# Hydrology-IFH/roger

Measured on AMD Instinct MI355X. Metric: cell-timesteps/sec on SVAT_benchmark grid, higher is better.
Workload: dtype f64

## Files before the change

include/roger_hip.h:

```cpp
#ifndef ROGER_HIP_H
#define ROGER_HIP_H

#include <stddef.h>
#include <stdint.h>

#ifdef __cplusplus
extern "C" {
#endif

#define RH_ABI_VERSION 6
#define RH_SLOTS_PER_DAY 144

typedef enum rh_status {
    RH_OK = 0,
    RH_ERR_ARG = -1,
    RH_ERR_HIP = -2,
    RH_ERR_STATE = -3,
    RH_ERR_NODEVICE = -4
} rh_status;

typedef enum rh_plane {
#define RH_FIELD_1(name) RH_P_##name,
#define RH_FIELD_2(name) RH_P_##name, RH_P_##name##_m1,
#define RH_FIELD(name, type, levels) RH_FIELD_##levels(name)
// ... 81 lines not shown
int rh_snow(rh_ctx *ctx);
int rh_infiltration(rh_ctx *ctx);
int rh_subsurface_runoff(rh_ctx *ctx);
int rh_surface_routing(rh_ctx *ctx);
int rh_subsurface_routing(rh_ctx *ctx);
int rh_step_routed(rh_ctx *ctx, int monthly);
int rh_route_out(rh_ctx *ctx, int which);
int rh_route_in(rh_ctx *ctx, int which);
int rh_route_get_edges(rh_ctx *ctx, int which, double *q_lo, double *q_hi);
int rh_route_get_static_edges(rh_ctx *ctx, int32_t *flow_dir_lo, int32_t *flow_dir_hi, int32_t *mask_lo, int32_t *mask_hi);
int rh_route_set_halo(rh_ctx *ctx, int side, const double *q, const int32_t *flow_dir, const int32_t *mask);
int rh_capillary_rise(rh_ctx *ctx);
int rh_storage(rh_ctx *ctx);
int rh_num_error(rh_ctx *ctx);
int rh_after_timestep(rh_ctx *ctx);
int rh_step_core(rh_ctx *ctx);

int rh_step_phase1(rh_ctx *ctx);
int rh_step_phase2(rh_ctx *ctx);
int rh_step_phase3(rh_ctx *ctx, int monthly);
int rh_svat_step(rh_ctx *ctx, int monthly);
int rh_svat_step_scalars(rh_ctx *ctx, int monthly, rh_scalars *s);
int rh_param_stats(rh_ctx *ctx, double *derived_fraction, double *uniform_bytes_per_cell);
int rh_step_summary(rh_ctx *ctx);
int rh_step_finish(rh_ctx *ctx, int monthly);
int rh_step_summary_expand(rh_ctx *ctx, int32_t *dev_dst64);
int rh_step_finish_compress(rh_ctx *ctx, int monthly, const int32_t *dev_src64);
int rh_set_forcing_stations(rh_ctx *ctx, const double *prec, const double *ta, const double *pet, const int64_t *year, const int64_t *month,
                            const int64_t *doy, int64_t nitt_forc, int n_stations, const int32_t *station_index);
int rh_hooks_phase(rh_ctx *ctx);
int rh_run_steps(rh_ctx *ctx, int64_t nsteps);
int rh_plane_is_pure_output(int model, int plane);
int rh_set_time_limit(rh_ctx *ctx, int64_t t_end);
int64_t rh_sparse_steps(const rh_ctx *ctx);
void *rh_predicate_words(rh_ctx *ctx);
int rh_predicates_expand(rh_ctx *ctx, int word, int32_t *dev_dst64);
int rh_predicates_compress(rh_ctx *ctx, int word, const int32_t *dev_src64);

int rh_comm_unique_id(void *id128);
int rh_comm_init(rh_ctx *ctx, const void *id128, int nranks, int rank);
int rh_set_comm(rh_ctx *ctx, void *nccl_comm);
int rh_comm_set_grid(rh_ctx *ctx, int px, int py);
int rh_comm_info(rh_ctx *ctx, int *nranks, int *rank);
int rh_run_steps_dist(rh_ctx *ctx, int64_t nsteps);

int rh_diag_configure(rh_ctx *ctx, const int *rate_planes, int n_rate, const int *collect_planes, int n_collect, int n_slots);
// ... 26 lines not shown
```

roger_amd/_native.py:

```python
import ctypes as C
import os

import numpy as np

PKG = os.path.dirname(os.path.abspath(__file__))
LIB_PATH = os.environ.get("ROGER_HIP_LIB", os.path.join(PKG, "libroger_hip.so"))


ABI_VERSION = 6


class RhConfig(C.Structure):
    _fields_ = [("nx", C.c_int64), ("ny", C.c_int64), ("device", C.c_int32), ("enable_lateral_flow", C.c_int32)] + [
        (k, C.c_double) for k in (
            "pi", "r_mp", "l_sc", "sf", "ta_fm", "rmax", "transp_water_stress", "atol", "rtol", "clay_min",
            "clay_max", "theta_rew_min", "theta_rew_max", "rew_min", "rew_max", "z_evap_max", "zroot_to_zsoil_max",
            "a_bc", "b_bc")
    ] + [("end_event", C.c_int64), ("hpi", C.c_int64), ("dx", C.c_double), ("placement_probes", C.c_int32), ("enable_routing_1D", C.c_int32),
         ("dy", C.c_double)]


class RhScalars(C.Structure):
    _fields_ = [
        ("itt", C.c_int64), ("time", C.c_int64), ("dt_secs", C.c_int64), ("itt_day", C.c_int64),
# ... 103 lines not shown
    lib.rh_step_routed.argtypes = [vp, i32]
    lib.rh_planes_held.argtypes = [vp]
    lib.rh_route_out.argtypes = [vp, i32]
    lib.rh_route_in.argtypes = [vp, i32]
    lib.rh_route_get_edges.argtypes = [vp, i32, vp, vp]
    lib.rh_route_get_static_edges.argtypes = [vp, vp, vp, vp, vp]
    lib.rh_route_set_halo.argtypes = [vp, i32, vp, vp, vp]
    lib.rh_diag_set_interval.argtypes = [vp, i64]
    lib.rh_diag_slot_times.argtypes = [vp, i32, C.POINTER(C.c_int64), C.POINTER(C.c_int64)]
    lib.rh_step_summary_expand.argtypes = [vp, vp]
    lib.rh_step_finish_compress.argtypes = [vp, i32, vp]
    lib.rh_set_forcing_weights.argtypes = [vp, vp, vp, vp]
    lib.rh_diag_configure.argtypes = [vp, vp, i32, vp, i32, i32]
    lib.rh_diag_download.argtypes = [vp, i32, i32, vp, C.c_size_t]
    lib.rh_diag_steps.argtypes = [vp, i32, C.POINTER(C.c_int64)]
    lib.rh_diag_device_ptr.argtypes = [vp, i32, i32]
    lib.rh_diag_device_ptr.restype = vp
    lib.rh_points_configure.argtypes = [vp, vp, i32, vp, i32, i64]
    lib.rh_points_count.argtypes = [vp, C.POINTER(C.c_int64)]
    lib.rh_points_read.argtypes = [vp, i64, i64, vp, vp, C.c_size_t]
    lib.rh_svat_step.argtypes = [vp, i32]
    lib.rh_svat_step_scalars.argtypes = [vp, i32, C.POINTER(RhScalars)]
    lib.rh_param_stats.argtypes = [vp, C.POINTER(C.c_double), C.POINTER(C.c_double)]
    lib.rh_run_steps.argtypes = [vp, i64]
    lib.rh_set_forcing_series.argtypes = [vp, vp, vp, vp, vp, vp, vp, i64]
    lib.rh_predicates_expand.argtypes = [vp, i32, vp]
    lib.rh_predicates_compress.argtypes = [vp, i32, vp]
    lib.rh_calibrate_copy.argtypes = [vp, i32, i32, i32]
    lib.rh_selftest_pow.argtypes = [vp, vp, vp, i64]
    lib.rh_selftest_window_sum.argtypes = [vp, vp, i64, vp]
    lib.rh_debug_swap_arenas.argtypes = [vp, vp]
    lib.rh_predicate_words.argtypes = [vp]
    lib.rh_predicate_words.restype = vp
    lib.rh_timing_summary.argtypes = [vp, C.POINTER(C.c_double), C.POINTER(C.c_int64)]
    lib.rh_timing_detail.argtypes = [vp, C.POINTER(C.c_double), C.POINTER(C.c_int32), C.c_int64, C.POINTER(C.c_int64)]
    lib.rh_enable_timing.argtypes = [vp, i32]
    _declare_sas(lib)
    _lib = lib
    return lib


class RhSasConfig(C.Structure):
    _fields_ = [("n_cells", C.c_int64), ("ages", C.c_int32), ("substeps", C.c_int32), ("device", C.c_int32),
                ("forcing_days", C.c_int32), ("age_statistics", C.c_int32), ("keep_distributions", C.c_int32),
                ("vsmow", C.c_double), ("d18O_min", C.c_double), ("d18O_max", C.c_double),
                ("tracer", C.c_int32), ("solver", C.c_int32)]
# ... 184 lines not shown


def sas_selftest_pow(x, k):
    lib = load()
    x = np.ascontiguousarray(x, dtype=np.float64)
    k = np.ascontiguousarray(np.broadcast_to(k, x.shape), dtype=np.float64)
    out = np.empty_like(x)
    rc = lib.rh_sas_selftest_pow(x.ctypes.data_as(C.c_void_p), k.ctypes.data_as(C.c_void_p), out.ctypes.data_as(C.c_void_p), x.size)
    if rc != 0:
        raise NativeError(f"rh_sas_selftest_pow failed ({rc})")
    return out


DAILY_INPUTS = ("inf_mat_rz", "inf_pf_rz", "inf_pf_ss", "evap_soil", "transp", "q_rz", "q_ss", "cpr_rz", "C_in")


DECLARED_SYMBOLS = (
    "rh_default_config", "rh_create", "rh_destroy", "rh_last_error", "rh_abi_version", "rh_set_stream", "rh_sync",
    "rh_num_planes", "rh_plane_name", "rh_plane_is_int", "rh_plane_index", "rh_num_cells", "rh_upload",
    "rh_download", "rh_plane_device_ptr", "rh_set_scalars", "rh_get_scalars", "rh_set_luts", "rh_set_forcing_day",
    "rh_topo", "rh_params_surface", "rh_params_soil", "rh_initial_conditions", "rh_adaptive_dt", "rh_interception",
    "rh_evapotranspiration", "rh_snow", "rh_infiltration", "rh_subsurface_runoff", "rh_capillary_rise",
    "rh_storage", "rh_num_error", "rh_after_timestep", "rh_step_phase1", "rh_step_phase2", "rh_step_phase3",
    "rh_svat_step", "rh_svat_step_scalars", "rh_param_stats", "rh_predicate_words", "rh_timing_summary", "rh_timing_detail", "rh_enable_timing", "rh_set_forcing_series",
    "rh_hooks_phase", "rh_run_steps", "rh_predicates_expand", "rh_predicates_compress", "rh_step_core", "rh_calibrate_copy", "rh_debug_swap_arenas", "rh_selftest_pow", "rh_selftest_window_sum", "rh_set_lut_mlms", "rh_params_lateral",
    "rh_step_summary", "rh_step_finish", "rh_diag_set_interval", "rh_diag_slot_times", "rh_placement_report", "rh_step_summary_expand", "rh_step_finish_compress", "rh_diag_configure", "rh_diag_download", "rh_diag_device_ptr", "rh_diag_steps",
    "rh_set_forcing_weights", "rh_adaptive_dt_finish", "rh_diag_upload", "rh_diag_set_slot_state", "rh_set_forcing_stations", "rh_step_mode", "rh_comm_unique_id", "rh_comm_init", "rh_set_comm", "rh_comm_info", "rh_comm_set_grid", "rh_plane_is_pure_output", "rh_sparse_steps", "rh_set_time_limit", "rh_run_steps_dist",
    "rh_surface_routing", "rh_subsurface_routing", "rh_step_routed", "rh_planes_held", "rh_route_out", "rh_route_in", "rh_route_get_edges", "rh_route_get_static_edges", "rh_route_set_halo",
    "rh_points_configure", "rh_points_count", "rh_points_read",
)


def selftest_window_sum(v144, itd):
    lib = load()
    v = np.ascontiguousarray(v144, dtype=np.float64)
    t = np.ascontiguousarray(itd, dtype=np.int64)
    if v.size != 144:
        raise ValueError("selftest_window_sum: a series of 144 slots")
    out = np.empty(2 * t.size, dtype=np.float64)
    rc = lib.rh_selftest_window_sum(v.ctypes.data_as(C.c_void_p), t.ctypes.data_as(C.c_void_p), t.size, out.ctypes.data_as(C.c_void_p))
    if rc != 0:
        raise NativeError(f"rh_selftest_window_sum failed ({rc})")
    return out[0::2], out[1::2]


def selftest_pow(x, y):
    lib = load()
# ... 237 lines not shown
        return n.value

    def points_read(self, first, n):
        n = int(n)
        nv, nc = getattr(self, "_points_shape", (0, 0))
        hdr = np.empty((n, 3), dtype=np.int64)
        values = np.empty((n, nv, nc), dtype=np.float64)
        self._check(self._lib.rh_points_read(self._h, int(first), n, hdr.ctypes.data_as(C.c_void_p), values.ctypes.data_as(C.c_void_p),
                                             values.nbytes), "rh_points_read")
        return hdr, values

    def pure_output_planes(self):
        model = 2 if self.routing else int(self.lateral)
        return [nm for nm, p in self.index.items() if self._lib.rh_plane_is_pure_output(model, p) == 1]

    def set_time_limit(self, t_end):
        self._check(self._lib.rh_set_time_limit(self._h, -1 if t_end is None else int(t_end)), "rh_set_time_limit")

    def param_stats(self):
        d, u = C.c_double(), C.c_double()
        self._check(self._lib.rh_param_stats(self._h, C.byref(d), C.byref(u)), "rh_param_stats")
        return d.value, u.value

    def sparse_steps(self):
        return int(self._lib.rh_sparse_steps(self._h))

    def step_mode(self):
        m = self._lib.rh_step_mode(self._h)
        return bool(m & 1), bool(m & 2)

    def comm_init(self, unique_id, nranks, rank):
        buf = C.create_string_buffer(bytes(unique_id), 128)
        self._check(self._lib.rh_comm_init(self._h, buf, int(nranks), int(rank)), "rh_comm_init")

    def comm_init_torch(self, group=None):
        import torch.distributed as dist

        rank, world = (dist.get_rank(group), dist.get_world_size(group)) if dist.is_initialized() else (0, 1)
        box = [comm_unique_id() if rank == 0 else None]
        if world > 1:
            dist.broadcast_object_list(box, src=0, group=group)
        self.comm_init(box[0], world, rank)

    def comm_info(self):
        n, r = C.c_int(), C.c_int()
        self._check(self._lib.rh_comm_info(self._h, C.byref(n), C.byref(r)), "rh_comm_info")
# ... 58 lines not shown
```

roger_amd/csrc/rh_context.h:

```cpp
#pragma once
struct DeviceHolds {
    bool pmask_valid = false;
    bool rot_consistent = false, m1_stale = false;
    bool summary_valid = false;
    bool routed_summary = false;
    bool exch_valid = false;
    bool pending_valid = false;
    bool pre_valid = false;
    int pending_hooks = 0;
    bool sparse_next = false;
    bool outputs_stale = false;
    bool last_sparse = false;
    bool agg_daily_stale = true;
    bool pred_daily_stale = true;
    bool front_daily_stale = true;
    int last_front = 0;
};

struct Switches {
    bool lazy_ok, sparse_ok, tail_ok, routed_device_ok, defer_select_ok, cell_front_ok;
    int64_t cell_front_max, cell_agg_split_min;
    int pmask_flags, placement_probes;
};
static Switches read_switches(const rh_config &cfg) {
    auto unset = [](const char *name) { return std::getenv(name) == nullptr; };
    auto number = [](const char *name, long long dflt) { const char *v = std::getenv(name); return v ? std::atoll(v) : dflt; };
    Switches s;
    s.lazy_ok = unset("RH_NO_LAZY_ROTATION");
    s.sparse_ok = unset("RH_NO_SPARSE_STORES");
    s.tail_ok = unset("RH_NO_TAIL_CTRL");
    s.routed_device_ok = unset("RH_ROUTED_BY_ROUTINE");
    s.defer_select_ok = unset("RH_NO_DEFERRED_SELECT");
    s.cell_front_ok = unset("RH_PER_CELL_OLD_FRONT") && s.defer_select_ok;
    s.cell_front_max = number("RH_CELL_FRONT_MAX", 2097152);
    s.cell_agg_split_min = number("RH_CELL_AGG_SPLIT_MIN", 65536);
    s.pmask_flags = (unset("RH_NO_PARAM_UNIFORM") ? 1 : 0) | (unset("RH_NO_PARAM_DERIVE") ? 2 : 0) | (unset("RH_NO_MASK_CONSTANT") ? 4 : 0);
    s.placement_probes = (int)number("RH_PLACEMENT_PROBES", cfg.placement_probes);
    return s;
}

struct rh_ctx {
    Stream stream;
    rh_config cfg = {};
    int64_t n = 0;
    Arena arena = {};
    DevBuf<char> arena_mem;
    DevBuf<DevState> dev;
    PinnedBlock<HostExport> hexp;
    unsigned long long hexp_seq = 0;
    DevBuf<unsigned long long> pmask_buf;
    DevBuf<double> forc_cell_buf[3];
    DevBuf<double> weight_buf[3];
    DevBuf<int> station_buf;
    DevBuf<double> forc_multi_buf;
    DevBuf<double> transpose_buf;
    DevBuf<double> agg_cell_buf;
    DevBuf<char> series_buf;
    DevBuf<double> mlms_buf;
    DevBuf<void> stage_buf;
    bool per_cell = false;
    bool forcing_set = false;
    DeviceHolds held;
    Switches sw;
    int n_groups = 1;
    bool obs_reads_m1 = false;
    bool obs_reads_sparse = false;
    int64_t t_end = -1;
    int64_t call_sparse_steps = 0;
    DevBuf<double> diag_buf;
    DevBuf<long long> diag_steps_buf;
    long long diag_interval = 86400;
    int diag_n = 0, diag_slots = 0;
    int diag_planes[32] = {};
// ... 76 lines not shown

template <class M, class V>
static hipError_t dev_put(rh_ctx *ctx, M DevState::*member, const V &v) {
    static_assert(sizeof(M) == sizeof(V), "the host value must have the member's size");
    return hipMemcpyAsync(&(ctx->dev.get()->*member), &v, sizeof(M), hipMemcpyHostToDevice, ctx->stream);
}
template <class M>
static hipError_t dev_zero(rh_ctx *ctx, M DevState::*member) {
    return hipMemsetAsync(&(ctx->dev.get()->*member), 0, sizeof(M), ctx->stream);
}

static void materialise_m1(rh_ctx *ctx) {
    if (!ctx->held.m1_stale) return;
    hipLaunchKernelGGL(k_rotate_all, dim3(grid_for(ctx->n)), dim3(RH_BLOCK), 0, ctx->stream, ctx->arena);
    ctx->held.m1_stale = false;
}
static void control_inputs_changed(rh_ctx *ctx, bool on_device = false) {
    ctx->held.pending_valid = ctx->held.pre_valid = false;
    if (on_device) ctx->held.exch_valid = false;
}
static void planes_touched(rh_ctx *ctx) {
    materialise_m1(ctx);
    ctx->held.pmask_valid = false;
    ctx->held.rot_consistent = false;
    ctx->held.summary_valid = false;
    ctx->held.routed_summary = false;
    control_inputs_changed(ctx, true);
}
static void summary_path_left(rh_ctx *ctx) {
    ctx->held.summary_valid = false;
    control_inputs_changed(ctx, true);
}
static void cell_forcing_changed(rh_ctx *ctx) {
    ctx->held.agg_daily_stale = true;
    ctx->held.pred_daily_stale = true;
    ctx->held.front_daily_stale = true;
}
static void front_takes_over(rh_ctx *ctx, int kind) {
    if (ctx->held.last_front != kind) {
        if (kind == 1) ctx->held.agg_daily_stale = ctx->held.pred_daily_stale = true;
        else ctx->held.front_daily_stale = true;
    }
    ctx->held.last_front = kind;
}
static void sparse_step_enqueued(rh_ctx *ctx, bool sparse) {
    ctx->held.outputs_stale = ctx->held.last_sparse = sparse;
    ctx->call_sparse_steps += sparse ? 1 : 0;
}
static void fused_step_enqueued(rh_ctx *ctx, int flags, bool lazy, bool sparse, bool exch) {
    ctx->held.rot_consistent = true;
    ctx->held.m1_stale = lazy;
    sparse_step_enqueued(ctx, sparse);
    ctx->held.summary_valid = !(flags & RH_TAIL_SKIP);
    ctx->held.pending_valid = (flags & RH_TAIL_CTRL) != 0;
    ctx->held.pre_valid = (flags & RH_TAIL_PRE) && !(flags & RH_TAIL_CTRL);
    ctx->held.pending_hooks = (flags & RH_TAIL_HOOKS) != 0;
    ctx->held.exch_valid = exch;
}
static void routed_step_enqueued(rh_ctx *ctx, bool sparse) {
    ctx->held.routed_summary = true;
    sparse_step_enqueued(ctx, sparse);
}

#define LAUNCH_CELLS(ctx, kern)                                                                                          \
    do {                                                                                                                 \
        planes_touched(ctx);                                                                                             \
        hipLaunchKernelGGL(kern, dim3(grid_for((ctx)->n)), dim3(RH_BLOCK), 0, (ctx)->stream, (ctx)->arena, (ctx)->dev); \
    } while (0)
#define LAUNCH_PRED(ctx, kern)                                                                                           \
    do {                                                                                                                 \
        planes_touched(ctx);                                                                                             \
        hipLaunchKernelGGL(kern, dim3((ctx)->pred_blocks), dim3(RH_BLOCK), 0, (ctx)->stream, (ctx)->arena, (ctx)->dev, 0); \
    } while (0)
#define LAUNCH_ONE(ctx, kern, ...) hipLaunchKernelGGL(kern, dim3(1), dim3(64), 0, (ctx)->stream, __VA_ARGS__)
// ... 28 lines not shown
```

roger_amd/csrc/rh_dev_state.h:

```cpp
#ifndef RH_DEV_STATE_H
#define RH_DEV_STATE_H

#define RH_BLOCK 256
#ifndef RH_STRIDE_PAD
#define RH_STRIDE_PAD 0
#endif
#define RH_PRED_BLOCKS 1024
#define RH_DONE_GROUPS 256
#define RH_DONE_STRIDE 32
#define RH_DEVERR_FORCING 1u
#define RH_TAIL_USE_NEXT 1
#define RH_TAIL_CTRL 2
#define RH_TAIL_HOOKS 4
#define RH_TAIL_PRE 16
#define RH_TAIL_SKIP 8
#define RH_SRC_WORD3 0
#ifndef RH_WSTRIDE
#define RH_WSTRIDE 16
#endif
#define RH_SRC_SUMW 1
#define RH_POINTS_MAX_CELLS 256
#define RH_POINTS_MAX_PLANES 32
#ifndef RH_STEP_WAVES
#define RH_STEP_WAVES 2
#endif

struct DevState {
    Consts K;
    rh_scalars S;
    StepCtx X;
    unsigned long long words[4];
    unsigned long long bflags[2][RH_PRED_BLOCKS];
    unsigned long long day_bflags[RH_PRED_BLOCKS];
    int pred_blocks;
    unsigned long long sumw[64 * RH_WSTRIDE];
    unsigned int done_grp[RH_DONE_GROUPS * RH_DONE_STRIDE];
    unsigned int done_top;
    unsigned long long sanity_last;
// ... 22 lines not shown
    const int64_t *calendar[3];
    int64_t nitt_forc;
    long long t_end;
    int skipped;
    int monthly;
    const double *weights[3];
    int n_stations;
    const int *station_idx;
    double *forc_multi;

    const unsigned long long *pmask;

    const double *mlms;
    int64_t mlms_rows;
    int max_slope_per;
    Luts L;

    double *points;
    long long *points_hdr;
    long long points_rows, points_cap;
    int points_ncells, points_nplanes;
    int points_planes[RH_POINTS_MAX_PLANES];
    long long points_cells[RH_POINTS_MAX_CELLS];
};

struct HostExport {
    rh_scalars S;
    unsigned long long bad, bad_last;
    unsigned int err, pad;
    unsigned long long seq;
};

RH_DEV void wave_or_to(unsigned long long *word, unsigned long long bits) {
    for (int off = 32; off; off >>= 1) bits |= __shfl_xor(bits, off);
    if ((threadIdx.x & 63) == 0 && bits) {
        const unsigned long long seen = __hip_atomic_load(word, __ATOMIC_RELAXED, __HIP_MEMORY_SCOPE_AGENT);
        if (bits & ~seen) atomicOr(word, bits);
    }
}
RH_DEV void block_or_store(unsigned long long *slot, unsigned long long bits) {
    __shared__ unsigned long long wv[RH_BLOCK / 64];
    for (int off = 32; off; off >>= 1) bits |= __shfl_xor(bits, off);
    if ((threadIdx.x & 63) == 0) wv[threadIdx.x >> 6] = bits;
    __syncthreads();
    if (threadIdx.x == 0) {
        unsigned long long b = 0;
// ... 148 lines not shown
```

roger_amd/csrc/rh_setup.h:

```cpp
#pragma once
int rh_abi_version(void) { return RH_ABI_VERSION; }

void rh_default_config(rh_config *cfg) {
    std::memset(cfg, 0, sizeof(*cfg));
    cfg->nx = cfg->ny = 1;
    cfg->pi = 3.14159265358979323846264338327950588;
    cfg->r_mp = 2.5;
    cfg->l_sc = 10000;
    cfg->sf = 3;
    cfg->ta_fm = 0;
    cfg->rmax = 30;
    cfg->transp_water_stress = 0.75;
    cfg->atol = 1e-2;
    cfg->rtol = 1e-2;
    cfg->clay_min = 0.01;
    cfg->clay_max = 0.71;
    cfg->theta_rew_min = 0.02;
    cfg->theta_rew_max = 0.24;
    cfg->rew_min = 2;
    cfg->rew_max = 12;
    cfg->z_evap_max = 150;
    cfg->zroot_to_zsoil_max = 0.7;
    cfg->a_bc = 2;
    cfg->b_bc = 2;
// ... 91 lines not shown
        }
        if (ev0) (void)hipEventDestroy(ev0);
        if (ev1) (void)hipEventDestroy(ev1);
        size_t pick = 0;
        for (size_t k = 1; k < cand.size(); ++k)
            if (cand_ms[k] < cand_ms[pick]) pick = k;
        ctx->arena_mem = std::move(cand[pick]);
        ctx->arena.base = ctx->arena_mem;
        if (probes > 1) {
            ctx->probe_ms.push_back(cand_ms[pick]);
            for (size_t k = 0; k < cand.size(); ++k)
                if (k != pick) ctx->probe_ms.push_back(cand_ms[k]);
        }
    }
    if ((e = ctx->stage_buf.alloc((size_t)ctx->n * sizeof(double))) != hipSuccess) return bail(e, "hipMalloc(staging plane)");
    if ((e = ctx->dev.alloc(sizeof(DevState))) != hipSuccess) return bail(e, "hipMalloc(DevState)");
    if ((e = ctx->hexp.alloc()) != hipSuccess) return bail(e, "hipHostMalloc(scalar export block)");
    if ((e = hipMemsetAsync(ctx->dev, 0, sizeof(DevState), ctx->stream)) != hipSuccess) return bail(e, "hipMemset");
    {
        const size_t words = ((size_t)ctx->n + 63) / 64;
        if ((e = ctx->pmask_buf.alloc(words * sizeof(unsigned long long))) != hipSuccess) return bail(e, "hipMalloc(parameter words)");
        if ((e = hipMemsetAsync(ctx->pmask_buf, 0, words * sizeof(unsigned long long), ctx->stream)) != hipSuccess) return bail(e, "hipMemset");
        if ((e = dev_put(ctx, &DevState::pmask, *ctx->pmask_buf.addr())) != hipSuccess) return bail(e, "hipMemcpy(pmask)");
        if ((e = hipStreamSynchronize(ctx->stream)) != hipSuccess) return bail(e, "hipStreamSynchronize");
    }
    {
        static const long long no_limit = -1;
        if ((e = dev_put(ctx, &DevState::t_end, no_limit)) != hipSuccess) return bail(e, "hipMemcpy(t_end)");
    }
    Consts K;
    K.pi = cfg->pi; K.r_mp = cfg->r_mp; K.l_sc = cfg->l_sc; K.sf = cfg->sf; K.ta_fm = cfg->ta_fm; K.rmax = cfg->rmax;
    K.transp_water_stress = cfg->transp_water_stress; K.atol = cfg->atol; K.rtol = cfg->rtol;
    K.clay_min = cfg->clay_min; K.clay_max = cfg->clay_max; K.theta_rew_min = cfg->theta_rew_min;
    K.theta_rew_max = cfg->theta_rew_max; K.rew_min = cfg->rew_min; K.rew_max = cfg->rew_max;
    K.z_evap_max = cfg->z_evap_max; K.zroot_to_zsoil_max = cfg->zroot_to_zsoil_max; K.a_bc = cfg->a_bc; K.b_bc = cfg->b_bc;
    K.end_event = cfg->end_event; K.hpi = cfg->hpi;
    K.dx = cfg->dx; K.lateral = cfg->enable_lateral_flow ? 1 : 0;
    K.dy = cfg->dy; K.routing = cfg->enable_routing_1D ? 1 : 0;
    if ((e = dev_put(ctx, &DevState::K, K)) != hipSuccess) return bail(e, "hipMemcpy(Consts)");
    rh_scalars S;
    std::memset(&S, 0, sizeof(S));
    S.dt = 1;
    S.dt_secs = 3600;
    S.event_id_counter = 1;
    S.year[0] = S.year[1] = 1900;
    S.month[0] = S.month[1] = 1;
// ... 195 lines not shown
```

roger_amd/csrc/rh_step.h:

```cpp
#ifndef RH_STEP_H
#define RH_STEP_H

#define LD(name) rh_ld(a, RH_P_##name, i, c.name);
#define ST(name) rh_st(a, RH_P_##name, i, c.name);

constexpr int rh_param_bit(int plane) {
    switch (plane) {
#define RH_PB(name, bit) case RH_P_##name: return bit;
        RH_PARAM_BITS(RH_PB)
#undef RH_PB
        default: return -1;
    }
}
constexpr bool rh_param_derived(int plane) {
    switch (plane) {
#define RH_PD(name) case RH_P_##name:
        RH_DERIVED_FIELDS(RH_PD)
#undef RH_PD
        return true;
        default: return false;
    }
}
#if defined(RH_CENSUS)
#ifndef RH_CENSUS_PMASK
#define RH_CENSUS_PMASK 0ull
#endif
#endif
template <int PLANE, bool MK1, typename T>
RH_DEV void rh_ld_p(const Arena &a, int64_t i, T &dst, unsigned long long um) {
    constexpr int bit = rh_param_bit(PLANE);
    if constexpr (MK1 && PLANE == RH_P_maskCatch) {
        dst = 1;
    } else if constexpr (bit < 0) {
        rh_ld(a, PLANE, i, dst);
    } else {
        if constexpr (rh_param_derived(PLANE)) {
            if (um >> 63) return;
        }
        const bool uni = (um >> bit) & 1ull;
        const int tile = __builtin_amdgcn_readfirstlane((int)(i >> RH_TILE_SHIFT));
        const int piece = __builtin_amdgcn_readfirstlane((int)(i & (RH_TILE_CELLS - 1)) & ~63);
        const T *p = reinterpret_cast<const T *>(a.base + (size_t)tile * a.stride + (size_t)PLANE * RH_SLOT_BYTES) + piece + (uni ? 0 : (int)(i & 63));
        dst = __builtin_nontemporal_load(p);
    }
}
#define LDP(name) rh_ld_p<RH_P_##name, MK1>(a, i, c.name, um);
RH_DEV unsigned long long bits_of(double v) { return (unsigned long long)__double_as_longlong(v); }
RH_DEV unsigned long long bits_of(int v) { return (unsigned long long)(unsigned)v; }
__global__ __launch_bounds__(RH_BLOCK) void k_param_mask(Arena a, DevState *D, unsigned long long *out, int flags) {
    const int64_t i = (int64_t)blockIdx.x * RH_BLOCK + threadIdx.x;
    const bool active = i < a.n;
    const int64_t ii = active ? i : a.n - 1;
    if ((int64_t)blockIdx.x * RH_BLOCK + (threadIdx.x & ~63) >= a.n) return;
    Col c;
    unsigned long long um = 0;
#define RH_PU(name, bit)                                                                                       \
    {                                                                                                          \
        rh_ld(a, RH_P_##name, ii, c.name);                                                                     \
        const unsigned long long mine = bits_of(c.name);                                                       \
        const unsigned long long first = ((unsigned long long)(unsigned)__builtin_amdgcn_readfirstlane((int)(mine >> 32)) << 32) | \
                                         (unsigned)__builtin_amdgcn_readfirstlane((int)mine);                  \
        if (__ballot(active && mine != first) == 0) um |= 1ull << bit;                                         \
    }
    RH_PARAM_BITS(RH_PU)
#undef RH_PU
    unsigned long long in_bits = 0, mon_bits = 0;
#define RH_PB(name, bit) const unsigned long long pbit_##name = 1ull << bit;
    RH_PARAM_BITS(RH_PB)
#undef RH_PB
#define RH_PI(name) in_bits |= pbit_##name;
    RH_PARAM_MONTHLY_INPUTS(RH_PI)
// ... 18 lines not shown
}
#define ROT(name) rh_st(a, RH_P_##name##_m1, i, c.name);

#define AL(xm1, x) c.xm1 = c.x;
#define RH_LOADS(seq, rt)                                          \
    if constexpr (LAZY) {                                          \
        RH_SEQ_##seq##_LLOAD_##rt(LDP) RH_SEQ_##seq##_ALIAS_##rt(AL) \
    } else {                                                       \
        RH_SEQ_##seq##_LOAD_##rt(LD)                               \
    }
#define RH_DERIVE(rt)                        \
    if constexpr (LAZY) {                    \
        if (um >> 63) rd_##rt(c, K);         \
        rl_##rt(c, K);                       \
    }
#ifdef RH_CENSUS
#define STK(name)
#else
#define STK(name) \
    if ((keepw[RH_P_##name >> 6] >> (RH_P_##name & 63)) & 1ull) rh_st(a, RH_P_##name, i, c.name);
#endif
#define RH_STORES(seq, rt)                                               \
    if constexpr (LAZY && SPARSE) {                                      \
        RH_SEQ_##seq##_SSTORE_##rt(ST)                                   \
        if constexpr (KEEP) { RH_SEQ_##seq##_KSTORE_##rt(STK) }          \
    } else if constexpr (LAZY) {                                         \
        RH_SEQ_##seq##_LSTORE_##rt(ST)                                   \
    } else {                                                             \
        RH_SEQ_##seq##_STORE_##rt(ST) RH_SEQ_##seq##_ROT_##rt(ROT)       \
    }
#define RH_PIN __builtin_amdgcn_sched_barrier(0);
#ifdef RH_STEP_PHASES
__device__ unsigned long long g_step_phases[256 * 64];
#define RH_PH(k)                                                                          \
    if ((threadIdx.x & 63) == 0) {                                                        \
        const unsigned long long t_ = clock64();                                          \
        atomicAdd(&g_step_phases[(blockIdx.x & 255) * 64 + ph_cls * 20 + (k)], t_ - ph_t);                          \
        ph_t = t_;                                                                        \
    }
#else
#define RH_PH(k)
#endif
#define RH_STEP_BODY(seq, mon_rt, MON_LOADS, MON_RUN, sub_rt, sub_call, ne_rt, ne_call, at_rt, at_call) \
    RH_LOADS(seq, rt_select_prec) RH_LOADS(seq, rt_select_pet) MON_LOADS RH_LOADS(seq, rt_interception) RH_PIN  \
    rt_select_prec(c, X, prec_s, ta_s); RH_STORES(seq, rt_select_prec)                                                \
    rt_select_pet(c, X, pet_v, ta_v); RH_STORES(seq, rt_select_pet) RH_PH(1)                                      \
    q = summary_bits_pt(c.prec, c.ta, K);                                                                \
    MON_RUN                                                                                              \
    RH_LOADS(seq, rt_evapotranspiration) RH_PIN                                                                 \
    rt_interception(c, K); RH_STORES(seq, rt_interception) RH_PH(2)                                               \
// ... 14 lines not shown
    rt_inf_finish(c, K, X); RH_STORES(seq, rt_inf_finish) RH_PH(9)                                                \
    RH_LOADS(seq, rt_capillary_rise) RH_PIN                                                                     \
    RH_DERIVE(sub_rt) sub_call; RH_STORES(seq, sub_rt) RH_PH(10)                                                   \
    RH_LOADS(seq, rt_storage) RH_PIN                                                                            \
    rt_capillary_rise(c, X); RH_STORES(seq, rt_capillary_rise) RH_PH(11)                                           \
    RH_LOADS(seq, ne_rt) RH_PIN                                                                                 \
    RH_DERIVE(rt_storage) rt_storage(c, X); RH_STORES(seq, rt_storage) RH_PH(12)                                   \
    RH_LOADS(seq, at_rt) RH_PIN                                                                                 \
    bad = ne_call; RH_STORES(seq, ne_rt) RH_PH(13)                                                                 \
    at_call; RH_STORES(seq, at_rt) RH_PH(14)

RH_DEV void post_summary(DevState *D, unsigned long long q, unsigned &dep) {
    unsigned long long qq = 0;
#pragma unroll
    for (int b = 0; b <= QB_P_NE0; ++b) qq |= __ballot((q >> b) & 1ull) ? (1ull << b) : 0ull;
    if ((threadIdx.x & 63) == 0 && qq) {
        const unsigned long long old = __hip_atomic_fetch_or(&D->sumw[(blockIdx.x & 63) * RH_WSTRIDE], qq, __ATOMIC_RELAXED, __HIP_MEMORY_SCOPE_AGENT);
        dep |= (unsigned)(old >> 63);
    }
}

template <bool MONTHLY, bool LATERAL, bool LAZY, bool SPARSE, bool KEEP = false, bool MK1 = false>
RH_DEV void step_column(const Arena &a, DevState *D, const StepCtx *Xp, int64_t i, unsigned long long &q, bool &bad, unsigned &dep, unsigned long long um,
                        bool post) {
    {
    const Consts K = D->K;
    const StepCtx X = *Xp;
    Col c;
    double pet_v = X.pet_sel_w, ta_v = X.ta_sel_w;
    double prec_s = X.prec_sel, ta_s = X.ta_sel;
    unsigned long long keepw[(RH_NPLANES + 63) / 64];
#pragma unroll
    for (int k = 0; k < (RH_NPLANES + 63) / 64; ++k) keepw[k] = KEEP ? D->keep[k] : 0ull;
#ifdef RH_STEP_PHASES
    const int ph_cls = X.dt < 0.5 ? 0 : (X.dt < 12 ? 1 : 2);
    unsigned long long ph_t = clock64();
    if ((threadIdx.x & 63) == 0) atomicAdd(&g_step_phases[(blockIdx.x & 255) * 64 + ph_cls * 20 + 19], 1ull);
#endif
#ifndef RH_CENSUS
    if (D->per_cell && X.sel_w >= 0) {
        pet_v = cell_agg(D, a.n, i, 3 * X.sel_w + 2);
        ta_v = cell_agg(D, a.n, i, 3 * X.sel_w + 1);
    }
    if (X.apply_sel == 2 && D->per_cell && X.sel_p >= 0) {
        prec_s = cell_agg(D, a.n, i, 3 * X.sel_p);
        ta_s = cell_agg(D, a.n, i, 3 * X.sel_p + 1);
    }
// ... 13 lines not shown
    } else {
        RH_STEP_BODY(step, , , , rt_subsurface_runoff, rt_subsurface_runoff(c, X), rt_num_error, rt_num_error(c, K),
                     rt_after_timestep, rt_after_timestep(c))
    }
    }
}

template <int MODE, bool LATERAL, bool LAZY, bool SPARSE = false, bool KEEP = false>
__global__ __launch_bounds__(RH_BLOCK, RH_STEP_WAVES) void k_step(Arena a, DevState *D, int flags, int n_groups, int *dst64) {
    const unsigned nb = gridDim.x - ((flags & RH_TAIL_PRE) ? 1u : 0u);
    const bool extra = blockIdx.x >= nb;
    const unsigned x = blockIdx.x & 7u, base_cnt = nb >> 3, rem = nb & 7u;
    const unsigned blk = x * base_cnt + (x < rem ? x : rem) + (blockIdx.x >> 3);
    const int64_t i = extra ? a.n : (int64_t)blk * RH_BLOCK + threadIdx.x;
    __shared__ unsigned wg_done;
    __shared__ CtrlLds tail_lds;
    const StepCtx *Xp = (flags & RH_TAIL_USE_NEXT) ? &D->X_next : &D->X;
#ifndef RH_CENSUS
    const bool halted = Xp->halt != 0;
    if (blockIdx.x == 0 && threadIdx.x == 0) {
        D->skipped = halted ? 1 : 0;
        if (halted) log_dt(D, 0);
    }
    if (halted) return;
#endif
    if (threadIdx.x == 0) wg_done = 0;
    __syncthreads();
    unsigned long long q = 0;
    bool bad = false;
    unsigned dep = 1;
    const bool post = !(flags & RH_TAIL_SKIP);
    if (i < a.n) {
        const bool monthly = MODE == 1 || (MODE == 2 && D->monthly != 0);
        unsigned long long um = 0;
        if constexpr (LAZY) {
#ifdef RH_CENSUS
            um = RH_CENSUS_PMASK;
#else
            const unsigned long long *pm = D->pmask;
            const unsigned long long w = pm ? pm[__builtin_amdgcn_readfirstlane((int)(i >> 6))] : 0ull;
            um = ((unsigned long long)(unsigned)__builtin_amdgcn_readfirstlane((int)(w >> 32)) << 32) | (unsigned)__builtin_amdgcn_readfirstlane((int)w);
#endif
        }
        const bool mk1 = LAZY && ((um >> 62) & 1ull);
#ifdef RH_CENSUS
        if (SPARSE) {
#else
        if (SPARSE && !Xp->last) {
#endif
            if (monthly) step_column<true, LATERAL, LAZY, SPARSE, KEEP>(a, D, Xp, i, q, bad, dep, um, post);
            else if (mk1) step_column<false, LATERAL, LAZY, SPARSE, KEEP, LAZY>(a, D, Xp, i, q, bad, dep, um, post);
            else step_column<false, LATERAL, LAZY, SPARSE, KEEP>(a, D, Xp, i, q, bad, dep, um, post);
        } else {
            if (monthly) step_column<true, LATERAL, LAZY, false>(a, D, Xp, i, q, bad, dep, um, post);
            else step_column<false, LATERAL, LAZY, false>(a, D, Xp, i, q, bad, dep, um, post);
        }
    } else if (post) {
        post_summary(D, 0ull, dep);
    }
#ifndef RH_CENSUS
    if (__builtin_expect(extra && threadIdx.x < 64, 0)) pre_tail(D, tail_lds, flags, dep);
#endif
    const bool any_bad = __any(bad);
    if (!post) {
        if (any_bad && (threadIdx.x & 63) == 0) __hip_atomic_fetch_or(&D->words[2], 1ull, __ATOMIC_RELAXED, __HIP_MEMORY_SCOPE_AGENT);
        return;
    }
    bool last = false;
    if ((threadIdx.x & 63) == 0) {
        if (any_bad) dep |= (unsigned)(__hip_atomic_fetch_or(&D->words[2], 1ull, __ATOMIC_RELAXED, __HIP_MEMORY_SCOPE_AGENT) >> 63);
        const unsigned o = atomicAdd(&wg_done, dep);
        if (o == (RH_BLOCK / 64) - 1) last = grid_completion(D, n_groups);
    }
#ifndef RH_CENSUS
    if (__shfl((int)last, 0)) step_tail(D, tail_lds, flags, dst64);
#endif
}

#ifdef RH_CENSUS
// ... 70 lines not shown
```

roger_amd/csrc/rh_stepping.h:

```cpp
#pragma once
static int timing_pair(rh_ctx *ctx, hipEvent_t *ev0, hipEvent_t *ev1) {
    if (!ctx->timing) return RH_OK;
    if (ctx->events.used + 2 > 2 * (size_t)RH_DT_LOG_CAP)
        return fail(ctx, RH_ERR_STATE, "timing: more than 65536 timed steps since rh_enable_timing(1); read the timings and enable again");
    HIPCHK(ctx, ctx->events.next_pair(ev0, ev1));
    return RH_OK;
}

#define SIMPLE_ENTRY(fname, kern)           \
    int fname(rh_ctx *ctx) {                \
        if (!ctx) return RH_ERR_ARG;        \
        LAUNCH_CELLS(ctx, kern);            \
        CHECK_LAUNCH(ctx);                  \
        return RH_OK;                       \
    }

SIMPLE_ENTRY(rh_topo, k_topo)
SIMPLE_ENTRY(rh_params_surface, k_params_surface)
SIMPLE_ENTRY(rh_params_soil, k_params_soil)
SIMPLE_ENTRY(rh_initial_conditions, k_initial_conditions)
SIMPLE_ENTRY(rh_interception, k_interception)
SIMPLE_ENTRY(rh_evapotranspiration, k_evapotranspiration)
SIMPLE_ENTRY(rh_snow, k_snow)
SIMPLE_ENTRY(rh_capillary_rise, k_capillary_rise)
// ... 96 lines not shown
}

using StepKernel = void (*)(Arena, DevState *, int, int, int *);
static StepKernel step_kernel(int mode, bool lateral, bool lazy, bool sparse, bool keep) {
#define RH_K4(M) {{k_step<M, true, true>, k_step<M, true, false>}, {k_step<M, false, true>, k_step<M, false, false>}}
    static const StepKernel sparse2[2][2] = {{k_step<2, true, true, true, true>, k_step<2, false, true, true, true>},
                                             {k_step<2, true, true, true>, k_step<2, false, true, true>}};
    static const StepKernel plain[3][2][2] = {RH_K4(2), RH_K4(1), RH_K4(0)};
#undef RH_K4
    return sparse ? sparse2[!keep][!lateral] : plain[2 - mode][!lateral][!lazy];
}
static int launch_fused_kernel(rh_ctx *ctx, int monthly, int flags = 0, int *dst64 = nullptr) {
    hipEvent_t ev0 = nullptr, ev1 = nullptr;
    if (int rc = timing_pair(ctx, &ev0, &ev1)) return rc;
    if (flags & RH_TAIL_CTRL) flags |= RH_TAIL_PRE;
    const dim3 grid(grid_for(ctx->n) + ((flags & RH_TAIL_PRE) ? 1u : 0u)), block(RH_BLOCK);
    const bool lat = ctx->cfg.enable_lateral_flow != 0;
    const bool lazy = ctx->sw.lazy_ok && ctx->held.rot_consistent && !ctx->obs_reads_m1;
    const bool sparse = lazy && ctx->held.sparse_next && monthly < 0;
    const bool keep = sparse && ctx->obs_reads_sparse;
    ctx->held.sparse_next = false;
    if (lazy)
        if (int rc = form_param_mask(ctx, grid)) return rc;
    hipExtLaunchKernelGGL(step_kernel(monthly < 0 ? 2 : (monthly ? 1 : 0), lat, lazy, sparse, keep), grid, block, 0, ctx->stream, ev0, ev1, 0,
                          ctx->arena, ctx->dev.get(), flags, ctx->n_groups, dst64);
    CHECK_LAUNCH(ctx);
    if (ctx->timing) ctx->events.taken();
    fused_step_enqueued(ctx, flags, lazy, sparse, dst64 != nullptr);
    return launch_observers(ctx, 1, grid.x);
}

static void launch_pred1(rh_ctx *ctx) {
    hipLaunchKernelGGL(k_pred1, dim3(ctx->pred_blocks), dim3(RH_BLOCK), 0, ctx->stream, ctx->arena, ctx->dev, ctx->held.pred_daily_stale ? 1 : 0);
    ctx->held.pred_daily_stale = false;
}
int rh_step_phase1(rh_ctx *ctx) {
    if (!ctx) return RH_ERR_ARG;
    if (int rc = need_forcing(ctx)) return rc;
    planes_touched(ctx);
    front_takes_over(ctx, 1);
    launch_pred1(ctx);
    LAUNCH_WG(ctx, k_reduce, ctx->dev, 0);
    CHECK_LAUNCH(ctx);
    return RH_OK;
}
static void launch_cell_agg(rh_ctx *ctx) {
// ... 295 lines not shown
```

roger_amd/csrc/rh_tools.h:

```cpp
#pragma once
int rh_predicates_expand(rh_ctx *ctx, int word, int32_t *dev_dst64) {
    if (!ctx || word < 0 || word > 3 || !dev_dst64) return RH_ERR_ARG;
    hipLaunchKernelGGL(k_words_expand, dim3(1), dim3(64), 0, ctx->stream, ctx->dev, word, dev_dst64);
    CHECK_LAUNCH(ctx);
    return RH_OK;
}
int rh_predicates_compress(rh_ctx *ctx, int word, const int32_t *dev_src64) {
    if (!ctx || word < 0 || word > 3 || !dev_src64) return RH_ERR_ARG;
    hipLaunchKernelGGL(k_words_compress, dim3(1), dim3(64), 0, ctx->stream, ctx->dev, word, dev_src64);
    CHECK_LAUNCH(ctx);
    return RH_OK;
}

int rh_calibrate_copy(rh_ctx *ctx, int src_plane0, int dst_plane0, int nplanes) {
    if (!ctx || nplanes <= 0 || src_plane0 < 0 || dst_plane0 < 0 || src_plane0 + nplanes > ctx->planes_held ||
        dst_plane0 + nplanes > ctx->planes_held)
        return RH_ERR_ARG;
    for (int p = 0; p < nplanes; ++p)
        if (PLANE_IS_INT[src_plane0 + p] || PLANE_IS_INT[dst_plane0 + p]) return fail(ctx, RH_ERR_ARG, "calibration planes must be float64");
    planes_touched(ctx);
    hipLaunchKernelGGL(k_calib_copy, dim3(grid_for(ctx->n)), dim3(RH_BLOCK), 0, ctx->stream, ctx->arena, src_plane0, dst_plane0, nplanes);
    CHECK_LAUNCH(ctx);
    return RH_OK;
}

int rh_debug_swap_arenas(rh_ctx *a, rh_ctx *b) {
    if (!a || !b || a->n != b->n || a->arena.stride != b->arena.stride || a->planes_held != b->planes_held) return RH_ERR_ARG;
    HIPCHK(a, hipStreamSynchronize(a->stream));
    HIPCHK(b, hipStreamSynchronize(b->stream));
    std::swap(a->arena_mem, b->arena_mem);
    std::swap(a->arena.base, b->arena.base);
    a->held.pmask_valid = b->held.pmask_valid = false;
    return RH_OK;
}

int rh_selftest_pow(const double *x, const double *y, double *out, int64_t n) {
    if (!x || !y || !out || n <= 0) return RH_ERR_ARG;
    double *d = nullptr;
    if (hipMalloc((void **)&d, (size_t)n * 3 * sizeof(double)) != hipSuccess) return RH_ERR_HIP;
    int rc = RH_OK;
    if (hipMemcpy(d, x, (size_t)n * sizeof(double), hipMemcpyHostToDevice) != hipSuccess ||
        hipMemcpy(d + n, y, (size_t)n * sizeof(double), hipMemcpyHostToDevice) != hipSuccess)
        rc = RH_ERR_HIP;
    if (rc == RH_OK) {
        hipLaunchKernelGGL(k_selftest_rh_pow, dim3((unsigned)((n + 255) / 256)), dim3(256), 0, 0, d, d + n, d + 2 * n, n);
        if (hipGetLastError() != hipSuccess || hipDeviceSynchronize() != hipSuccess ||
            hipMemcpy(out, d + 2 * n, (size_t)n * sizeof(double), hipMemcpyDeviceToHost) != hipSuccess)
            rc = RH_ERR_HIP;
    }
    (void)hipFree(d);
    return rc;
}

int rh_selftest_window_sum(const double *v144, const int64_t *itd, int64_t n, double *out2n) {
    if (!v144 || !itd || !out2n || n <= 0) return RH_ERR_ARG;
// ... 40 lines not shown
    HIPCHK(ctx, hipMemcpyAsync(w.data(), ctx->pmask_buf, words * sizeof(unsigned long long), hipMemcpyDeviceToHost, ctx->stream));
    HIPCHK(ctx, hipStreamSynchronize(ctx->stream));
    unsigned long long f64_bits = 0, i32_bits = 0, derived_bits = 0;
#define RH_PB(name, bit) const unsigned long long pbit_##name = 1ull << bit;
    RH_PARAM_BITS(RH_PB)
#undef RH_PB
#define RH_PL(name) (PLANE_IS_INT[RH_P_##name] ? i32_bits : f64_bits) |= pbit_##name;
    if (ctx->cfg.enable_lateral_flow) { RH_PARAM_LOADED_ONED(RH_PL) } else { RH_PARAM_LOADED_SVAT(RH_PL) }
#undef RH_PL
#define RH_PD(name) derived_bits |= pbit_##name;
    RH_DERIVED_FIELDS(RH_PD)
#undef RH_PD
    double derived = 0, bytes = 0;
    for (size_t k = 0; k < words; ++k) {
        const bool der = (w[k] >> 63) & 1ull;
        derived += der ? 1 : 0;
        const unsigned long long u = w[k] & (der ? ~derived_bits : ~0ull);
        bytes += 8.0 * __builtin_popcountll(u & f64_bits) + 4.0 * __builtin_popcountll(u & i32_bits);
    }
    *derived_fraction = derived / (double)words;
    *uniform_bytes_per_cell = bytes / (double)words;
    return RH_OK;
}
int rh_step_mode(const rh_ctx *ctx) {
    if (!ctx) return 0;
    return (ctx->held.m1_stale ? RH_STEP_MODE_LAZY : 0) | (ctx->held.pending_valid ? RH_STEP_MODE_TAIL : 0) | (ctx->held.last_sparse ? RH_STEP_MODE_SPARSE : 0);
}

void *rh_predicate_words(rh_ctx *ctx) { return ctx ? (void *)ctx->dev->words : nullptr; }

int rh_enable_timing(rh_ctx *ctx, int on) {
    if (!ctx) return RH_ERR_ARG;
    ctx->timing = on != 0;
    ctx->events.restart();
    control_inputs_changed(ctx);
    if (on) HIPCHK(ctx, ctx->dt_log_buf.alloc_once(sizeof(int) * RH_DT_LOG_CAP));
    int *log = on ? ctx->dt_log_buf.get() : nullptr;
    const int cap = RH_DT_LOG_CAP, zero = 0;
    HIPCHK(ctx, dev_put(ctx, &DevState::dt_log, log));
    HIPCHK(ctx, dev_put(ctx, &DevState::dt_log_cap, cap));
    HIPCHK(ctx, dev_put(ctx, &DevState::dt_log_n, zero));
    HIPCHK(ctx, hipStreamSynchronize(ctx->stream));
    return RH_OK;
}
int rh_timing_detail(rh_ctx *ctx, double *kernel_ms, int32_t *dt_secs, int64_t cap, int64_t *launches) {
    if (!ctx || !kernel_ms || !dt_secs || !launches || cap < 0) return RH_ERR_ARG;
// ... 25 lines not shown
```

Before: 5.783 billion.

## Track per-wave all-zero state planes to skip their loads and stores

Adds a per-wavefront bitmask recording which of twenty state planes (snow, depressions, wetting front, event sums) were entirely zero after the previous step. The lazy step kernel then substitutes zero for those loads and, in the sparse path, skips storing planes that stay zero. This is meant to cut memory traffic for planes that are usually zero in dry or snow-free regions. In exchange every step pays a ballot per candidate store plus a mask read and write per wave, and correctness relies on invalidating the mask whenever planes are touched from the host.

```diff
diff --git a/include/roger_hip.h b/include/roger_hip.h
--- a/include/roger_hip.h
+++ b/include/roger_hip.h
@@ -127,6 +127,7 @@
 int rh_svat_step(rh_ctx *ctx, int monthly);
 int rh_svat_step_scalars(rh_ctx *ctx, int monthly, rh_scalars *s);
 int rh_param_stats(rh_ctx *ctx, double *derived_fraction, double *uniform_bytes_per_cell);
+int rh_zero_plane_stats(rh_ctx *ctx, int32_t *planes, int64_t *waves_zero, int cap);
 int rh_step_summary(rh_ctx *ctx);
 int rh_step_finish(rh_ctx *ctx, int monthly);
 int rh_step_summary_expand(rh_ctx *ctx, int32_t *dev_dst64);
diff --git a/roger_amd/_native.py b/roger_amd/_native.py
--- a/roger_amd/_native.py
+++ b/roger_amd/_native.py
@@ -149,6 +149,7 @@
     lib.rh_svat_step.argtypes = [vp, i32]
     lib.rh_svat_step_scalars.argtypes = [vp, i32, C.POINTER(RhScalars)]
     lib.rh_param_stats.argtypes = [vp, C.POINTER(C.c_double), C.POINTER(C.c_double)]
+    lib.rh_zero_plane_stats.argtypes = [vp, vp, vp, i32]
     lib.rh_run_steps.argtypes = [vp, i64]
     lib.rh_set_forcing_series.argtypes = [vp, vp, vp, vp, vp, vp, vp, i64]
     lib.rh_predicates_expand.argtypes = [vp, i32, vp]
@@ -379,7 +380,7 @@
     "rh_topo", "rh_params_surface", "rh_params_soil", "rh_initial_conditions", "rh_adaptive_dt", "rh_interception",
     "rh_evapotranspiration", "rh_snow", "rh_infiltration", "rh_subsurface_runoff", "rh_capillary_rise",
     "rh_storage", "rh_num_error", "rh_after_timestep", "rh_step_phase1", "rh_step_phase2", "rh_step_phase3",
-    "rh_svat_step", "rh_svat_step_scalars", "rh_param_stats", "rh_predicate_words", "rh_timing_summary", "rh_timing_detail", "rh_enable_timing", "rh_set_forcing_series",
+    "rh_svat_step", "rh_svat_step_scalars", "rh_param_stats", "rh_zero_plane_stats", "rh_predicate_words", "rh_timing_summary", "rh_timing_detail", "rh_enable_timing", "rh_set_forcing_series",
     "rh_hooks_phase", "rh_run_steps", "rh_predicates_expand", "rh_predicates_compress", "rh_step_core", "rh_calibrate_copy", "rh_debug_swap_arenas", "rh_selftest_pow", "rh_selftest_window_sum", "rh_set_lut_mlms", "rh_params_lateral",
     "rh_step_summary", "rh_step_finish", "rh_diag_set_interval", "rh_diag_slot_times", "rh_placement_report", "rh_step_summary_expand", "rh_step_finish_compress", "rh_diag_configure", "rh_diag_download", "rh_diag_device_ptr", "rh_diag_steps",
     "rh_set_forcing_weights", "rh_adaptive_dt_finish", "rh_diag_upload", "rh_diag_set_slot_state", "rh_set_forcing_stations", "rh_step_mode", "rh_comm_unique_id", "rh_comm_init", "rh_set_comm", "rh_comm_info", "rh_comm_set_grid", "rh_plane_is_pure_output", "rh_sparse_steps", "rh_set_time_limit", "rh_run_steps_dist",
@@ -663,6 +664,13 @@
         self._check(self._lib.rh_param_stats(self._h, C.byref(d), C.byref(u)), "rh_param_stats")
         return d.value, u.value
 
+    def zero_plane_stats(self):
+        k = self._lib.rh_zero_plane_stats(self._h, None, None, 0)
+        self._check(min(k, 0), "rh_zero_plane_stats")
+        planes, waves = np.zeros(k, np.int32), np.zeros(k, np.int64)
+        self._check(min(self._lib.rh_zero_plane_stats(self._h, planes.ctypes.data, waves.ctypes.data, k), 0), "rh_zero_plane_stats")
+        return {self.planes[int(p)][0]: int(w) for p, w in zip(planes, waves)}
+
     def sparse_steps(self):
         return int(self._lib.rh_sparse_steps(self._h))
 
diff --git a/roger_amd/csrc/rh_context.h b/roger_amd/csrc/rh_context.h
--- a/roger_amd/csrc/rh_context.h
+++ b/roger_amd/csrc/rh_context.h
@@ -1,6 +1,7 @@
 #pragma once
 struct DeviceHolds {
     bool pmask_valid = false;
+    bool zmask_valid = false;
     bool rot_consistent = false, m1_stale = false;
     bool summary_valid = false;
     bool routed_summary = false;
@@ -18,7 +19,7 @@
 };
 
 struct Switches {
-    bool lazy_ok, sparse_ok, tail_ok, routed_device_ok, defer_select_ok, cell_front_ok;
+    bool lazy_ok, sparse_ok, tail_ok, routed_device_ok, defer_select_ok, cell_front_ok, zero_planes_ok;
     int64_t cell_front_max, cell_agg_split_min;
     int pmask_flags, placement_probes;
 };
@@ -29,6 +30,7 @@
     s.lazy_ok = unset("RH_NO_LAZY_ROTATION");
     s.sparse_ok = unset("RH_NO_SPARSE_STORES");
     s.tail_ok = unset("RH_NO_TAIL_CTRL");
+    s.zero_planes_ok = unset("RH_NO_ZERO_PLANES");
     s.routed_device_ok = unset("RH_ROUTED_BY_ROUTINE");
     s.defer_select_ok = unset("RH_NO_DEFERRED_SELECT");
     s.cell_front_ok = unset("RH_PER_CELL_OLD_FRONT") && s.defer_select_ok;
@@ -49,6 +51,7 @@
     PinnedBlock<HostExport> hexp;
     unsigned long long hexp_seq = 0;
     DevBuf<unsigned long long> pmask_buf;
+    DevBuf<unsigned long long> zmask_buf;
     DevBuf<double> forc_cell_buf[3];
     DevBuf<double> weight_buf[3];
     DevBuf<int> station_buf;
@@ -171,6 +174,7 @@
 static void planes_touched(rh_ctx *ctx) {
     materialise_m1(ctx);
     ctx->held.pmask_valid = false;
+    ctx->held.zmask_valid = false;
     ctx->held.rot_consistent = false;
     ctx->held.summary_valid = false;
     ctx->held.routed_summary = false;
@@ -199,6 +203,7 @@
 static void fused_step_enqueued(rh_ctx *ctx, int flags, bool lazy, bool sparse, bool exch) {
     ctx->held.rot_consistent = true;
     ctx->held.m1_stale = lazy;
+    ctx->held.zmask_valid = lazy;
     sparse_step_enqueued(ctx, sparse);
     ctx->held.summary_valid = !(flags & RH_TAIL_SKIP);
     ctx->held.pending_valid = (flags & RH_TAIL_CTRL) != 0;
diff --git a/roger_amd/csrc/rh_dev_state.h b/roger_amd/csrc/rh_dev_state.h
--- a/roger_amd/csrc/rh_dev_state.h
+++ b/roger_amd/csrc/rh_dev_state.h
@@ -14,6 +14,7 @@
 #define RH_TAIL_HOOKS 4
 #define RH_TAIL_PRE 16
 #define RH_TAIL_SKIP 8
+#define RH_STEP_ZVALID 32
 #define RH_SRC_WORD3 0
 #ifndef RH_WSTRIDE
 #define RH_WSTRIDE 16
@@ -82,6 +83,8 @@
     int points_ncells, points_nplanes;
     int points_planes[RH_POINTS_MAX_PLANES];
     long long points_cells[RH_POINTS_MAX_CELLS];
+
+    unsigned long long *zmask;
 };
 
 struct HostExport {
diff --git a/roger_amd/csrc/rh_setup.h b/roger_amd/csrc/rh_setup.h
--- a/roger_amd/csrc/rh_setup.h
+++ b/roger_amd/csrc/rh_setup.h
@@ -137,6 +137,9 @@
         if ((e = ctx->pmask_buf.alloc(words * sizeof(unsigned long long))) != hipSuccess) return bail(e, "hipMalloc(parameter words)");
         if ((e = hipMemsetAsync(ctx->pmask_buf, 0, words * sizeof(unsigned long long), ctx->stream)) != hipSuccess) return bail(e, "hipMemset");
         if ((e = dev_put(ctx, &DevState::pmask, *ctx->pmask_buf.addr())) != hipSuccess) return bail(e, "hipMemcpy(pmask)");
+        if ((e = ctx->zmask_buf.alloc(words * sizeof(unsigned long long))) != hipSuccess) return bail(e, "hipMalloc(zero words)");
+        if ((e = hipMemsetAsync(ctx->zmask_buf, 0, words * sizeof(unsigned long long), ctx->stream)) != hipSuccess) return bail(e, "hipMemset");
+        if ((e = dev_put(ctx, &DevState::zmask, *ctx->zmask_buf.addr())) != hipSuccess) return bail(e, "hipMemcpy(zmask)");
         if ((e = hipStreamSynchronize(ctx->stream)) != hipSuccess) return bail(e, "hipStreamSynchronize");
     }
     {
diff --git a/roger_amd/csrc/rh_step.h b/roger_amd/csrc/rh_step.h
--- a/roger_amd/csrc/rh_step.h
+++ b/roger_amd/csrc/rh_step.h
@@ -44,9 +44,49 @@
         dst = __builtin_nontemporal_load(p);
     }
 }
-#define LDP(name) rh_ld_p<RH_P_##name, MK1>(a, i, c.name, um);
 RH_DEV unsigned long long bits_of(double v) { return (unsigned long long)__double_as_longlong(v); }
 RH_DEV unsigned long long bits_of(int v) { return (unsigned long long)(unsigned)v; }
+
+#define RH_ZERO_BITS(X)                                                                                                       \
+    X(swe, 0) X(swe_top, 1) X(swe_ground, 2) X(S_snow, 3) X(z0, 4) X(S_dep, 5) X(z_wf, 6) X(z_wf_t0, 7) X(z_wf_t1, 8) X(y_sc, 9) \
+    X(z_sc, 10) X(t_sat, 11) X(prec, 12) X(swe_top_tot, 13) X(S_int_top, 14) X(S_int_ground, 15) X(inf_mp_event_csum, 16)     \
+    X(inf_sc_event_csum, 17) X(inf_mat, 18) X(inf_mat_rz, 19)
+#define RH_ZERO_NBITS 20
+constexpr int rh_zero_bit(int plane) {
+    switch (plane) {
+#define RH_ZB(name, bit) case RH_P_##name: return bit;
+        RH_ZERO_BITS(RH_ZB)
+#undef RH_ZB
+        default: return -1;
+    }
+}
+template <int PLANE, bool MK1, typename T>
+RH_DEV void rh_ld_z(const Arena &a, int64_t i, T &dst, unsigned long long um, unsigned long long zm) {
+    constexpr int zb = rh_zero_bit(PLANE);
+    if constexpr (zb < 0) {
+        rh_ld_p<PLANE, MK1>(a, i, dst, um);
+    } else {
+        if ((zm >> zb) & 1ull) dst = 0;
+        else rh_ld(a, PLANE, i, dst);
+    }
+}
+template <int PLANE, bool SKIP, typename T>
+RH_DEV void rh_st_z(const Arena &a, int64_t i, T v, unsigned long long zm, unsigned long long &zo) {
+    constexpr int zb = rh_zero_bit(PLANE);
+#ifdef RH_CENSUS
+    rh_st(a, PLANE, i, v);
+#else
+    if constexpr (zb < 0) {
+        rh_st(a, PLANE, i, v);
+    } else {
+        const bool zero = __ballot(bits_of(v) != 0ull) == 0ull;
+        if (zero) zo |= 1ull << zb;
+        if (!(SKIP && zero && ((zm >> zb) & 1ull))) rh_st(a, PLANE, i, v);
+    }
+#endif
+}
+#define LDP(name) rh_ld_z<RH_P_##name, MK1>(a, i, c.name, um, zm);
+#define STZ(name) rh_st_z<RH_P_##name, LAZY && SPARSE>(a, i, c.name, zm, zo);
 __global__ __launch_bounds__(RH_BLOCK) void k_param_mask(Arena a, DevState *D, unsigned long long *out, int flags) {
     const int64_t i = (int64_t)blockIdx.x * RH_BLOCK + threadIdx.x;
     const bool active = i < a.n;
@@ -111,10 +151,10 @@
 #endif
 #define RH_STORES(seq, rt)                                               \
     if constexpr (LAZY && SPARSE) {                                      \
-        RH_SEQ_##seq##_SSTORE_##rt(ST)                                   \
+        RH_SEQ_##seq##_SSTORE_##rt(STZ)                                  \
         if constexpr (KEEP) { RH_SEQ_##seq##_KSTORE_##rt(STK) }          \
     } else if constexpr (LAZY) {                                         \
-        RH_SEQ_##seq##_LSTORE_##rt(ST)                                   \
+        RH_SEQ_##seq##_LSTORE_##rt(STZ)                                  \
     } else {                                                             \
         RH_SEQ_##seq##_STORE_##rt(ST) RH_SEQ_##seq##_ROT_##rt(ROT)       \
     }
@@ -175,7 +215,7 @@
 
 template <bool MONTHLY, bool LATERAL, bool LAZY, bool SPARSE, bool KEEP = false, bool MK1 = false>
 RH_DEV void step_column(const Arena &a, DevState *D, const StepCtx *Xp, int64_t i, unsigned long long &q, bool &bad, unsigned &dep, unsigned long long um,
-                        bool post) {
+                        unsigned long long zm, unsigned long long &zo, bool post) {
     {
     const Consts K = D->K;
     const StepCtx X = *Xp;
@@ -235,7 +275,12 @@
         D->skipped = halted ? 1 : 0;
         if (halted) log_dt(D, 0);
     }
-    if (halted) return;
+    if (halted) {
+        if constexpr (LAZY) {
+            if (!(flags & RH_STEP_ZVALID) && i < a.n && (threadIdx.x & 63) == 0) D->zmask[i >> 6] = 0ull;
+        }
+        return;
+    }
 #endif
     if (threadIdx.x == 0) wg_done = 0;
     __syncthreads();
@@ -255,19 +300,33 @@
             um = ((unsigned long long)(unsigned)__builtin_amdgcn_readfirstlane((int)(w >> 32)) << 32) | (unsigned)__builtin_amdgcn_readfirstlane((int)w);
 #endif
         }
+        unsigned long long zm = 0, zo = 0;
+#ifndef RH_CENSUS
+        if constexpr (LAZY) {
+            if (flags & RH_STEP_ZVALID) {
+                const unsigned long long w = D->zmask[__builtin_amdgcn_readfirstlane((int)(i >> 6))];
+                zm = ((unsigned long long)(unsigned)__builtin_amdgcn_readfirstlane((int)(w >> 32)) << 32) | (unsigned)__builtin_amdgcn_readfirstlane((int)w);
+            }
+        }
+#endif
         const bool mk1 = LAZY && ((um >> 62) & 1ull);
 #ifdef RH_CENSUS
         if (SPARSE) {
 #else
         if (SPARSE && !Xp->last) {
 #endif
-            if (monthly) step_column<true, LATERAL, LAZY, SPARSE, KEEP>(a, D, Xp, i, q, bad, dep, um, post);
-            else if (mk1) step_column<false, LATERAL, LAZY, SPARSE, KEEP, LAZY>(a, D, Xp, i, q, bad, dep, um, post);
-            else step_column<false, LATERAL, LAZY, SPARSE, KEEP>(a, D, Xp, i, q, bad, dep, um, post);
+            if (monthly) step_column<true, LATERAL, LAZY, SPARSE, KEEP>(a, D, Xp, i, q, bad, dep, um, zm, zo, post);
+            else if (mk1) step_column<false, LATERAL, LAZY, SPARSE, KEEP, LAZY>(a, D, Xp, i, q, bad, dep, um, zm, zo, post);
+            else step_column<false, LATERAL, LAZY, SPARSE, KEEP>(a, D, Xp, i, q, bad, dep, um, zm, zo, post);
         } else {
-            if (monthly) step_column<true, LATERAL, LAZY, false>(a, D, Xp, i, q, bad, dep, um, post);
-            else step_column<false, LATERAL, LAZY, false>(a, D, Xp, i, q, bad, dep, um, post);
-        }
+            if (monthly) step_column<true, LATERAL, LAZY, false>(a, D, Xp, i, q, bad, dep, um, zm, zo, post);
+            else step_column<false, LATERAL, LAZY, false>(a, D, Xp, i, q, bad, dep, um, zm, zo, post);
+        }
+#ifndef RH_CENSUS
+        if constexpr (LAZY) {
+            if ((threadIdx.x & 63) == 0) D->zmask[i >> 6] = zo;
+        }
+#endif
     } else if (post) {
         post_summary(D, 0ull, dep);
     }
diff --git a/roger_amd/csrc/rh_stepping.h b/roger_amd/csrc/rh_stepping.h
--- a/roger_amd/csrc/rh_stepping.h
+++ b/roger_amd/csrc/rh_stepping.h
@@ -142,6 +142,7 @@
     ctx->held.sparse_next = false;
     if (lazy)
         if (int rc = form_param_mask(ctx, grid)) return rc;
+    if (lazy && ctx->held.zmask_valid && ctx->sw.zero_planes_ok) flags |= RH_STEP_ZVALID;
     hipExtLaunchKernelGGL(step_kernel(monthly < 0 ? 2 : (monthly ? 1 : 0), lat, lazy, sparse, keep), grid, block, 0, ctx->stream, ev0, ev1, 0,
                           ctx->arena, ctx->dev.get(), flags, ctx->n_groups, dst64);
     CHECK_LAUNCH(ctx);
diff --git a/roger_amd/csrc/rh_tools.h b/roger_amd/csrc/rh_tools.h
--- a/roger_amd/csrc/rh_tools.h
+++ b/roger_amd/csrc/rh_tools.h
@@ -31,6 +31,7 @@
     std::swap(a->arena_mem, b->arena_mem);
     std::swap(a->arena.base, b->arena.base);
     a->held.pmask_valid = b->held.pmask_valid = false;
+    a->held.zmask_valid = b->held.zmask_valid = false;
     return RH_OK;
 }
 
@@ -117,6 +118,30 @@
     *uniform_bytes_per_cell = bytes / (double)words;
     return RH_OK;
 }
+int rh_zero_plane_stats(rh_ctx *ctx, int32_t *planes, int64_t *waves_zero, int cap) {
+    if (!ctx) return RH_ERR_ARG;
+    static const int cand[RH_ZERO_NBITS] = {
+#define RH_ZB(name, bit) RH_P_##name,
+        RH_ZERO_BITS(RH_ZB)
+#undef RH_ZB
+    };
+    const size_t words = ((size_t)ctx->n + 63) / 64;
+    std::vector<unsigned long long> w(words, 0ull);
+    if (ctx->held.zmask_valid && ctx->sw.zero_planes_ok) {
+        if (hipMemcpyAsync(w.data(), ctx->zmask_buf, words * sizeof(unsigned long long), hipMemcpyDeviceToHost, ctx->stream) != hipSuccess ||
+            hipStreamSynchronize(ctx->stream) != hipSuccess)
+            return fail(ctx, RH_ERR_HIP, "rh_zero_plane_stats: reading the zero words failed");
+    }
+    for (int b = 0; b < RH_ZERO_NBITS && b < cap; ++b) {
+        if (planes) planes[b] = cand[b];
+        if (waves_zero) {
+            int64_t k = 0;
+            for (size_t j = 0; j < words; ++j) k += (w[j] >> b) & 1ull;
+            waves_zero[b] = k;
+        }
+    }
+    return RH_ZERO_NBITS;
+}
 int rh_step_mode(const rh_ctx *ctx) {
     if (!ctx) return 0;
     return (ctx->held.m1_stale ? RH_STEP_MODE_LAZY : 0) | (ctx->held.pending_valid ? RH_STEP_MODE_TAIL : 0) | (ctx->held.last_sparse ? RH_STEP_MODE_SPARSE : 0);
```

Result: slower. 5.379 billion (-7.0%).
